# NethermindEth/zinc

Hardware: AMD Instinct MI355X
Metric: Zip commit+open MCoeffs/s at 2^24 witness (higher is better)
Workload: dtype i64

## Files before the change

zinc_amd/csrc/kernels_commit.cuh:

```cuda
#pragma once
#include <hip/hip_runtime.h>
#include <stdint.h>

#include "blake3.cuh"

namespace zipk {

typedef __int128 i128;
typedef unsigned __int128 u128;

#ifdef ZIPK_DEBUG_STAMPS
constexpr uint32_t kStampRec = 64;
__device__ __forceinline__ unsigned long long stamp_hw_id() {
    const uint32_t xcc = __builtin_amdgcn_s_getreg((3 << 11) | 20), hw = __builtin_amdgcn_s_getreg((31 << 11) | 4);
    return (unsigned long long)xcc | ((unsigned long long)hw << 8);
}
#endif

struct CommitArgs {
    const int64_t *evals;
    const uint32_t *perm1;
    const uint32_t *perm2;
    uint64_t *rows;
    uint32_t compact_rows;
// ... 162 lines not shown
    template <int E0>
    __device__ __forceinline__ void store_row_of(uint32_t d0, uint32_t d1, uint32_t d2) {
        if (MASKED && !(smask & (1u << E0))) return;
        const uint32_t j = base + E0 * T + tid;
        const uint32_t s = (uint32_t)((int32_t)d2 >> 31);
        if (MODE == kStorePacked) {
            const uint32_t pos = pbase<E0>() + lanes_below(__builtin_amdgcn_ballot_w64(true));
            *reinterpret_cast<uint4 *>(pk_v + (size_t)pos * 64) = make_uint4(d0, d1, d2, s);
        } else if (compact) {
            *reinterpret_cast<uint4 *>(out_row + (size_t)j * 2) = make_uint4(d0, d1, d2, s);
        } else {
            uint4 *o = reinterpret_cast<uint4 *>(out_row + (size_t)j * 4);
            o[0] = make_uint4(d0, d1, d2, s);
            o[1] = make_uint4(s, s, s, s);
        }
    }
    template <int E0>
    __device__ __forceinline__ void store_row() {
        uint32_t d0, d1, d2;
        entry<E0>(d0, d1, d2);
        store_row_of<E0>(d0, d1, d2);
    }
    template <int E0>
    __device__ __forceinline__ void leaf(uint32_t (&h)[8]) {
        uint32_t d0, d1, d2;
        entry<E0>(d0, d1, d2);
        store_row_of<E0>(d0, d1, d2);
        blake3_leaf_sext96(d0, d1, d2, h);
        if (!MASKED || (smask & (0x100u << E0))) {
            if (MODE == kStorePacked) {
                const uint32_t pos = pbase<8 + E0>() + lanes_below(__builtin_amdgcn_ballot_w64(true));
                store_hash(reinterpret_cast<uint32_t *>(pk_n + pk_off0) + (size_t)pos * 32, h);
            } else {
                store_hash(tree + (size_t)(base + E0 * T + tid) * 8, h);
            }
        }
    }
    template <int LVL, int E0>
    __device__ __forceinline__ void store(const uint32_t (&h)[8]) {
        if (MASKED && LVL <= 2 && !(smask & ((LVL == 1 ? 0x10000u : 0x1000000u) << (E0 >> LVL)))) return;
        const uint32_t e = E0 + (tid & ((1u << LVL) - 1u));
        const uint32_t n = (base + e * T + tid) >> LVL;
        if (MODE == kStorePacked && LVL == 1) {
            const uint64_t act = __builtin_amdgcn_ballot_w64(true);
            const bool odd = tid & 1u;
            const uint32_t pos = (odd ? pbase<16 + (E0 >> 1) * 2 + 1>() : pbase<16 + (E0 >> 1) * 2>()) +
                                 lanes_below(act & (odd ? 0xAAAAAAAAAAAAAAAAull : 0x5555555555555555ull));
            store_hash(reinterpret_cast<uint32_t *>(pk_n + pk_off1) + (size_t)pos * 32, h);
        } else if (MODE == kStorePacked && LVL == 2) {
            const uint64_t act = __builtin_amdgcn_ballot_w64(true);
            const uint32_t q = tid & 3u;
            constexpr int K0 = 24 + ((E0 >> 2) & 1) * 4;
            const uint32_t b01 = (q & 1u) ? pbase<K0 + 1>() : pbase<K0>(), b23 = (q & 1u) ? pbase<K0 + 3>() : pbase<K0 + 2>();
            const uint32_t pos = ((q & 2u) ? b23 : b01) + lanes_below(act & (0x1111111111111111ull << q));
            store_hash(reinterpret_cast<uint32_t *>(pk_n + pk_off2) + (size_t)pos * 32, h);
        } else {
            store_hash(tree + ((size_t)level_off(cw, LVL) + n) * NW, h);
        }
    }
};

template <int E>
__device__ __forceinline__ uint32_t store_mask(const uint32_t *need, uint32_t cw, uint32_t base, uint32_t T, uint32_t tid) {
    if (!need) return 0xFFFFFFFFu;
    const uint32_t *nv = need, *n0 = nv + (cw + 31) / 32, *n1 = n0 + (cw + 31) / 32, *n2 = n1 + (cw / 2 + 31) / 32;
    uint32_t m = 0;
#pragma unroll
    for (int e = 0; e < E; e++) {
        const uint32_t j = base + e * T + tid;
        m |= ((nv[j >> 5] >> (j & 31)) & 1u) << e;
        m |= ((n0[j >> 5] >> (j & 31)) & 1u) << (8 + e);
    }
#pragma unroll
    for (int g = 0; g < E / 2; g++) {
        const uint32_t i = (base + (2 * g + (tid & 1u)) * T + tid) >> 1;
        m |= ((n1[i >> 5] >> (i & 31)) & 1u) << (16 + g);
    }
#pragma unroll
    for (int g = 0; g < E / 4; g++) {
        const uint32_t i = (base + (4 * g + (tid & 3u)) * T + tid) >> 2;
        m |= ((n2[i >> 5] >> (i & 31)) & 1u) << (24 + g);
    }
    return m;
}

template <int E, int E0, class Src>
__device__ __forceinline__ void store_rows_only(Src &src) {
    if constexpr (E0 < E) {
        src.template store_row<E0>();
        store_rows_only<E, E0 + 1>(src);
    }
}

template <int LVL, int E0, class Src>
__device__ __forceinline__ void bfly_hash(Src &src, uint32_t (&h)[8]) {
    if constexpr (LVL == 0) {
        src.template leaf<E0>(h);
    } else {
        uint32_t A[8], B[8], m[16];
        bfly_hash<LVL - 1, E0>(src, A);
        bfly_hash<LVL - 1, E0 + (1 << (LVL - 1))>(src, B);
        const bool up = (src.tid >> (LVL - 1)) & 1;
#pragma unroll
        for (int i = 0; i < 8; i++) {
            const uint32_t snd = up ? A[i] : B[i];
            const uint32_t rcv = __shfl_xor(snd, 1 << (LVL - 1), 64);
            m[i] = up ? rcv : A[i];
            m[8 + i] = up ? B[i] : rcv;
        }
        blake3_block64(m, h);
        src.template store<LVL, E0>(h);
    }
}

template <bool ILV>
__device__ __forceinline__ void upper_stage(const CommitArgs &a, uint32_t first, uint32_t nrows_c, uint32_t lvl, uint32_t nl,
                                            uint32_t lane, uint32_t nlanes) {
    constexpr uint32_t NW = kNodeWords<ILV>;
    const uint32_t cw = a.cw, depth = 31u - __builtin_clz(cw);
    const uint32_t u_shift = depth - (lvl - 1u) - nl;
    const uint32_t total = nrows_c << u_shift;
    const uint32_t slot0 = round_slot(blockIdx.x, gridDim.x, a.classes);
    for (uint32_t idx = lane; idx < total; idx += nlanes) {
        const uint32_t ri = idx >> u_shift, i = idx & ((1u << u_shift) - 1u);
        const uint32_t r = slot0 + (first + ri) * gridDim.x;
        uint32_t *tree = tree_of<ILV>(a.layers, cw, r);
        const uint32_t *ch = tree + ((size_t)level_off(cw, lvl - 1u) + ((size_t)i << nl)) * NW;
        uint32_t c0[8], c1[8], h0[8];
        load_hash(ch, c0);
        load_hash(ch + NW, c1);
        if (nl == 1u) {
            blake3_node(c0, c1, h0);
            store_hash(tree + ((size_t)level_off(cw, lvl) + i) * NW, h0);
            if (lvl == depth) store_hash(a.roots + (size_t)r * 8, h0);
        } else {
            uint32_t c2[8], c3[8], h1[8], h2[8];
            blake3_node(c0, c1, h0);
            uint32_t *o = tree + ((size_t)level_off(cw, lvl) + 2u * i) * NW;
            store_hash(o, h0);
            asm volatile("" ::: "memory");
            load_hash(ch + 2 * NW, c2);
            load_hash(ch + 3 * NW, c3);
            blake3_node(c2, c3, h1);
            store_hash(o + NW, h1);
            blake3_node(h0, h1, h2);
            store_hash(tree + ((size_t)level_off(cw, lvl + 1u) + i) * NW, h2);
            if (lvl + 1u == depth) store_hash(a.roots + (size_t)r * 8, h2);
        }
    }
}

struct ChunkCursor {
    uint32_t first = 0, index = 0;
    __device__ __forceinline__ bool ends_with(const CommitArgs &a, uint32_t round, bool last) const {
        if (last) return true;
        if (a.chunk_ends) return (a.chunk_ends >> round) & 1u;
        return (round + 1) % a.rounds_per_chunk == 0;
    }
    __device__ __forceinline__ void advance(uint32_t round) {
        first = round + 1;
        index++;
    }
};

constexpr uint32_t kFinisherFlagWords = 16;

// ... 106 lines not shown
            __syncthreads();
            uint4 *in = bufA, *out = bufB;
            for (uint32_t lvl = p_lvl; lvl <= depth; lvl++) {
                const uint32_t w = cw >> lvl, sh = 31u - __builtin_clz(w), m = p_nrows * w;
                for (uint32_t idx = tid; idx < m; idx += T) {
                    const uint32_t ri = idx >> sh, i = idx & (w - 1u);
                    const uint32_t r = slot0 + (p_first + ri) * gridDim.x;
                    const uint4 a0 = in[4u * idx], a1 = in[4u * idx + 1u], b0 = in[4u * idx + 2u], b1 = in[4u * idx + 3u];
                    const uint32_t c0[8] = {a0.x, a0.y, a0.z, a0.w, a1.x, a1.y, a1.z, a1.w};
                    const uint32_t c1[8] = {b0.x, b0.y, b0.z, b0.w, b1.x, b1.y, b1.z, b1.w};
                    uint32_t h[8];
                    blake3_node(c0, c1, h);
                    store_hash(tree_of<ILV>(a.layers, cw, r) + ((size_t)level_off(cw, lvl) + i) * NW, h);
                    if (lvl == depth) store_hash(a.roots + (size_t)r * 8, h);
                    out[2u * idx] = make_uint4(h[0], h[1], h[2], h[3]);
                    out[2u * idx + 1u] = make_uint4(h[4], h[5], h[6], h[7]);
                }
                __syncthreads();
                uint4 *t = in;
                in = out;
                out = t;
            }
            if (wave == 0u) publish(a, p_index, lane);
            return;
        }
        after_hash(a, wave, lane, T);
    }

    __device__ __forceinline__ void chunk_end(const CommitArgs &a, uint32_t first_level, const ChunkCursor &cc, uint32_t round,
                                              bool last, uint32_t tid, uint32_t T) {
        const uint32_t wave = __builtin_amdgcn_readfirstlane(tid >> 6), lane = tid & 63u;
        if (!HASH) {
            if (a.chunk_done) {
                __syncthreads();
                if (wave == 0) publish(a, cc.index, lane);
            }
            return;
        }
        const uint32_t cw = a.cw, depth = 31u - __builtin_clz(cw);
        const uint32_t first = cc.first, nrows_c = round - first + 1;
        uint32_t lvl = first_level;
        const bool now = last || lvl > depth;
        if (now) {
            __syncthreads();
            if (lvl <= depth) {
                const uint32_t nl = depth - lvl >= 1u ? 2u : 1u;
                upper_stage<ILV>(a, first, nrows_c, lvl, nl, tid, T);
                lvl += nl;
            }
        }
        if (depth == 0 && tid == 0) {
            for (uint32_t ri = 0; ri < nrows_c; ri++) {
                const uint32_t r = round_slot(blockIdx.x, gridDim.x, a.classes) + (first + ri) * gridDim.x;
                uint32_t h[8];
                load_hash(a.layers + (size_t)r * (2u * cw) * 8, h);
                store_hash(a.roots + (size_t)r * 8, h);
            }
        }
        if (!last) p_base = lvl;
        pending = true;
        p_first = first;
        p_nrows = nrows_c;
        p_lvl = lvl;
        p_index = cc.index;
    }
};

__device__ __forceinline__ void stamp_clock(const CommitArgs &a, int slot) {
    if (a.clock && blockIdx.x == 0 && threadIdx.x == 0) {
        a.clock[2 * slot] = __builtin_amdgcn_s_memtime();
        a.clock[2 * slot + 1] = __builtin_amdgcn_s_memrealtime();
    }
}

__device__ __forceinline__ uint32_t opaque_zero(uint32_t dep) {
    uint32_t z;
    asm volatile("s_mov_b32 %0, 0" : "=s"(z) : "s"(dep));
    return z;
}

template <int E, bool HASH, int MODE = kStoreAll>
__global__ void __launch_bounds__(1024, 4) raa_commit_kernel(CommitArgs a) {
    constexpr bool MASKED = MODE != kStoreAll;
    extern __shared__ __align__(16) unsigned char smem[];
    constexpr int LOGE = (E == 1) ? 0 : (E == 2) ? 1 : (E == 4) ? 2 : 3;
    static_assert((1 << LOGE) == E && E <= 8, "E must be 1, 2, 4 or 8");

    const uint32_t tid0 = threadIdx.x, T = blockDim.x;
    constexpr uint32_t PAD = 32 / E;
    const uint32_t PS = T + PAD;
    const uint32_t cw = a.cw, row_len = a.row_len;
    const bool active = tid0 < a.nact;
    stamp_clock(a, 0);

    i128 *wave_tot = reinterpret_cast<i128 *>(smem);
    uint64_t *t2lo = reinterpret_cast<uint64_t *>(smem + 512);
    uint32_t *t2hi = reinterpret_cast<uint32_t *>(t2lo + E * PS);
    int64_t *rowbuf = reinterpret_cast<int64_t *>(t2hi + E * PS);
    uint32_t pidx[E];
    auto load_pidx = [&](uint32_t t) {
#pragma unroll
        for (int e = 0; e < E; e++) {
            uint32_t v1 = 0, v2 = 0;
            if (active) {
                v1 = a.perm1[t * E + e] & (row_len - 1);
                const uint32_t p2 = a.perm2[t * E + e];
                v2 = (p2 & (E - 1)) * PS + (p2 >> LOGE);
            }
            pidx[e] = v1 | (v2 << 16);
        }
    };
    load_pidx(tid0);
    const uint32_t smask = (MASKED && active) ? store_mask<E>(a.need, cw, 0u, a.nact, tid0) : 0xFFFFFFFFu;
    uint32_t ptab[16] = {};
    if (MODE == kStorePacked) {
        const uint32_t *wt = a.pk_tab + (size_t)__builtin_amdgcn_readfirstlane(tid0 >> 6) * 16;
#pragma unroll
        for (int k = 0; k < 16; k++) ptab[k] = __builtin_amdgcn_readfirstlane(wt[k]);
    }
    constexpr int NPF = (E >= 2) ? E / 2 : 1;
    const bool prefetch = row_len == NPF * T;
    int64_t nxt[NPF];

#ifdef ZIPK_DEBUG_STAMPS
    unsigned long long ph_a = 0, ph_b = 0, ph_c = 0, ph_t;
    if (tid0 == 0 && a.stamps) {
        a.stamps[(size_t)kStampRec * blockIdx.x] = wall_clock64();
        a.stamps[(size_t)kStampRec * blockIdx.x + 2] = stamp_hw_id();
    }
#define ZIPK_PH(acc) do { const unsigned long long now_ = wall_clock64(); acc += now_ - ph_t; ph_t = now_; } while (0)
#else
#define ZIPK_PH(acc) do { } while (0)
#endif
    uint32_t round = 0;
    ChunkCursor cc;
    if (a.classes > 1u) {
        const uint32_t c = commit_class(blockIdx.x, gridDim.x, a.classes);
        cc.index = c;
        const uint32_t prio = (a.classes - 1u - c) * 3u / (a.classes - 1u);
        if (prio == 3u) __builtin_amdgcn_s_setprio(3);
        else if (prio == 2u) __builtin_amdgcn_s_setprio(2);
        else if (prio == 1u) __builtin_amdgcn_s_setprio(1);
    }
    ChunkFinisher<HASH, MODE == kStorePacked> fin;
    fin.init(reinterpret_cast<uint32_t *>(rowbuf + row_len), tid0);
    const uint32_t wave0 = __builtin_amdgcn_readfirstlane(tid0 >> 6);
    for (uint32_t row = round_slot(blockIdx.x, gridDim.x, a.classes); row < a.num_rows; row += gridDim.x, round++) {
#ifdef ZIPK_DEBUG_STAMPS
        ph_t = wall_clock64();
#endif
        const uint32_t z = opaque_zero(row);
        const uint32_t tid = tid0 + z;
        const int64_t *in = a.evals + (size_t)row * row_len;
        uint64_t *out_row = a.rows + (size_t)row * cw * (a.compact_rows ? 2 : 4);

        const bool has_next = row + gridDim.x < a.num_rows;
        if (!(prefetch && round)) {
            if (round) lds_barrier();
            for (uint32_t i = tid; i < row_len; i += T) rowbuf[i] = in[i];
            lds_barrier();
        }
        if (prefetch && has_next) {
            const int64_t *nin = a.evals + (size_t)(row + gridDim.x) * row_len;
#pragma unroll
            for (int k = 0; k < NPF; k++) nxt[k] = nin[k * T + tid];
        }

        i128 v[E];
        if (active) {
#pragma unroll
            for (int e = 0; e < E; e++) v[e] = (i128)rowbuf[(pidx[e] ^ z) & 0xFFFFu];
#pragma unroll
            for (int e = 1; e < E; e++) v[e] += v[e - 1];
        } else {
#pragma unroll
            for (int e = 0; e < E; e++) v[e] = 0;
        }
        {
            const i128 pre = block_exclusive_scan_i96(v[E - 1], wave_tot, 0);
            if (active) {
#pragma unroll
                for (int e = 0; e < E; e++) {
                    v[e] += pre;
                    const uint32_t slot = e * PS + tid;
                    t2lo[slot] = (uint64_t)v[e];
                    t2hi[slot] = (uint32_t)((u128)v[e] >> 64);
                }
            }
        }
        lds_barrier();
        if (active) {
#pragma unroll
            for (int e = 0; e < E; e++) {
                const uint32_t slot = (pidx[e] ^ z) >> 16;
                const uint64_t lo = t2lo[slot];
                const int64_t hi = (int64_t)(int32_t)t2hi[slot];
                v[e] = (i128)(((u128)(uint64_t)hi << 64) | lo);
            }
#pragma unroll
            for (int e = 1; e < E; e++) v[e] += v[e - 1];
        }
        {
            const i128 pre = block_exclusive_scan_i96(v[E - 1], wave_tot, 1);
#pragma unroll
            for (int e = 0; e < E; e++) v[e] += pre;
        }

        if (active) {
#pragma unroll
            for (int e = 0; e < E; e++) {
                const uint32_t slot = e * PS + tid;
                t2lo[slot] = (uint64_t)v[e];
                t2hi[slot] = (uint32_t)((u128)v[e] >> 64);
            }
        }
        if (prefetch && has_next) {
#pragma unroll
            for (int k = 0; k < NPF; k++) rowbuf[k * T + tid] = nxt[k];
        }
        fin.top_of_row();
        lds_barrier();
        ZIPK_PH(ph_a);
        if (active) {
            StridedLeaves<E, MODE, true> src;
            src.out_row = out_row;
            src.compact = a.compact_rows;
            src.tree = HASH ? tree_of<MODE == kStorePacked>(a.layers, cw, row) : nullptr;
            src.cw = cw;
            src.T = a.nact;
            src.tid = tid;
            src.smask = smask;
            if (MODE == kStorePacked) {
                src.set_packed(a, row);
#pragma unroll
                for (int k = 0; k < 16; k++) src.ptab[k] = ptab[k];
            }
            {
                const uint32_t slot0 = (tid & (E - 1)) * PS + (tid >> LOGE);
                src.lz_lo = t2lo + slot0;
                src.lz_hi = t2hi + slot0;
                src.lz_stride = a.nact >> LOGE;
            }
            if (HASH) {
                uint32_t top[8];
                bfly_hash<LOGE, 0>(src, top);
            } else {
                store_rows_only<E, 0>(src);
            }
        }
        ZIPK_PH(ph_b);
        fin.after_hash(a, wave0, tid0 & 63u, T);
        const bool last = row + gridDim.x >= a.num_rows;
        if (cc.ends_with(a, round, last)) {
            fin.chunk_end(a, LOGE + 1, cc, round, last, tid, T);
            cc.advance(round);
        }
        ZIPK_PH(ph_c);
#ifdef ZIPK_DEBUG_STAMPS
        if (tid0 == 0 && a.stamps && round < kStampRec - 8) a.stamps[(size_t)kStampRec * blockIdx.x + 8 + round] = ph_t;
#endif
    }
    fin.after_loop(a, wave0, tid0 & 63u, T, smem + 512, (uint32_t)(E * PS * 12u));
    stamp_clock(a, 1);
#ifdef ZIPK_DEBUG_STAMPS
    if (tid0 == 0 && a.stamps) {
        unsigned long long *o = a.stamps + (size_t)kStampRec * blockIdx.x;
        o[1] = wall_clock64();
        o[3] = ph_a; o[4] = ph_b; o[5] = ph_c; o[6] = round;
    }
#endif
}

constexpr size_t c16_lds_bytes(uint32_t T) {
    return 512 + (size_t)16 * (T + 2) * 8 + (size_t)16 * (T + 2) + (size_t)T * 4 + 64;
}

template <int B, int P = 0>
__device__ __forceinline__ void transpose8_stage(uint32_t (&x)[8], bool up) {
    if constexpr (P < 4) {
        constexpr int r = ((P >> B) << (B + 1)) | (P & ((1 << B) - 1)), r2 = r | (1 << B);
        const uint32_t lo = x[r], hi = x[r2];
        const uint32_t rcv = __shfl_xor(up ? lo : hi, 1 << B, 64);
        x[r] = up ? rcv : lo;
        x[r2] = up ? hi : rcv;
        transpose8_stage<B, P + 1>(x, up);
    }
}
__device__ __forceinline__ void transpose8(uint32_t (&x)[8], uint32_t lane) {
    transpose8_stage<0>(x, lane & 1u);
    transpose8_stage<1>(x, (lane >> 1) & 1u);
    transpose8_stage<2>(x, (lane >> 2) & 1u);
}

template <uint32_t T, bool HASH, int MODE = kStoreAll>
__global__ void __launch_bounds__(T, 4) raa_commit16_kernel(CommitArgs a) {
    constexpr bool MASKED = MODE != kStoreAll;
    static_assert(MODE == kStoreAll || MODE == kStoreHinted || MODE == kStorePacked, "store mode");
    extern __shared__ __align__(16) unsigned char smem[];
    constexpr int E = 16;
    constexpr uint32_t PS = T + 2;
    const uint32_t tid0 = threadIdx.x;
    const uint32_t cw = a.cw, row_len = a.row_len;
    stamp_clock(a, 0);

    i128 *wave_tot = reinterpret_cast<i128 *>(smem);
    uint64_t *t2lo = reinterpret_cast<uint64_t *>(smem + 512);
    int8_t *t2dh = reinterpret_cast<int8_t *>(t2lo + (size_t)E * PS);
    int32_t *ghi = reinterpret_cast<int32_t *>(t2dh + (size_t)E * PS);
    uint64_t *park_lo = reinterpret_cast<uint64_t *>(smem + 512);
    uint32_t *park_hi = reinterpret_cast<uint32_t *>(park_lo + (size_t)8 * PS);

    const uint32_t smask0 = MASKED ? store_mask<8>(a.need, cw, 0u, 16u, (tid0 & ~7u) * 16u + (tid0 & 7u)) : 0xFFFFFFFFu;
    const uint32_t smask1 = MASKED ? store_mask<8>(a.need, cw, 0u, 16u, (tid0 & ~7u) * 16u + 8u + (tid0 & 7u)) : 0xFFFFFFFFu;
    uint32_t ptab0[16] = {}, ptab1[16] = {};
    if (MODE == kStorePacked) {
        const uint32_t *wt = a.pk_tab + (size_t)__builtin_amdgcn_readfirstlane(tid0 >> 6) * 32;
#pragma unroll
        for (int k = 0; k < 16; k++) {
            ptab0[k] = __builtin_amdgcn_readfirstlane(wt[k]);
// ... 369 lines not shown
```

zinc_amd/csrc/zip_hip.hip:

```cpp
#include <hip/hip_runtime.h>
#include <dlfcn.h>
#include <algorithm>
#include <atomic>
#include <chrono>
#include <thread>

#include <climits>
#include <cstdarg>
#include <cstdio>
#include <cstdlib>
#include <cstring>
#include <functional>
#include <map>
#include <memory>
#include <mutex>
#include <new>
#include <string>
#include <vector>

#include "../../include/zip_hip.h"
#include "kernels_commit.cuh"
#include "kernels_open.cuh"
#include "kernels_batch.cuh"
#include "kernels_verify.cuh"
#include "kernels_batch_verify.cuh"
#include "kernels_sumcheck.cuh"
#include "kernels_sumcheck_tail.cuh"
#include "kernels_sumcheck_wide.cuh"
#include "kernels_spartan.cuh"
#include "rccl_dyn.h"

using namespace zipk;

namespace {

typedef unsigned __int128 u128;

bool is_pow2(uint64_t x) { return x && !(x & (x - 1)); }
uint32_t ilog2(uint64_t x) { return 63u - (uint32_t)__builtin_clzll(x); }

long env_long(const char *name, long def, long lo, long hi) {
    const char *e = getenv(name);
    if (!e) return def;
    char *end = nullptr;
    const long v = strtol(e, &end, 10);
    return end == e || v < lo || v > hi ? def : v;
}

struct KernelStat {
    uint32_t launches = 0;
    float total_ms = 0.f;
};
struct PendingEvent {
    const char *name;
    hipEvent_t start, stop;
};

}

struct PackedLayout {
    uint32_t stride = 0, off[3] = {};
};
struct HintPlan {
    uint32_t cw = 0, e = 0, threads = 0;
    bool want_packed = false;
    std::vector<uint32_t> cols;
    std::vector<uint32_t> bm;
    bool packed = false;
    PackedLayout L;
    std::vector<uint32_t> wave_tab;
    std::vector<uint16_t> pos[4];
    std::vector<uint16_t> own_ranks;
    unsigned char *dev = nullptr;
    std::function<void(unsigned char *)> release;
    HintPlan() = default;
    HintPlan(const HintPlan &) = delete;
    HintPlan &operator=(const HintPlan &) = delete;
    ~HintPlan() { if (dev && release) release(dev); }
    bool ranks(const uint32_t *cs, uint32_t n, uint16_t *out) const {
        for (uint32_t i = 0; i < n; i++) {
            const uint32_t col = cs[i];
            if (col >= cw) return false;
            const uint16_t r[4] = {pos[0][col], pos[1][col ^ 1u], pos[2][(col >> 1) ^ 1u], pos[3][(col >> 2) ^ 1u]};
            for (int k = 0; k < 4; k++) {
                if (r[k] == 0xFFFF) return false;
                out[4 * i + k] = r[k];
            }
        }
        return true;
    }
};

static inline int speculation_default_flag() {
    const long v = env_long("ZIP_HIP_SPECULATE", -1, 0, 1);
    return v < 0 ? 1 : v == 0 ? 0 : 2;
}

struct zip_ctx {
    zip_params p{};
    uint32_t depth = 0;
    uint32_t rows_local = 0;
    int device = 0;
    hipStream_t stream = nullptr, s_commit = nullptr, s_upper = nullptr;
    uint32_t n_chunks = 1;
    uint32_t knob_rpb = 0;
    int knob_stream = -1;
    std::string knob_chunk_rounds;
    bool no_compact = false;
    uint32_t num_cus = 256;
    uint32_t *timeout_flag_h = nullptr, *timeout_flag_d = nullptr;
    unsigned long long *clock_h = nullptr, *clock_d = nullptr;
    std::vector<hipEvent_t> dep_event_pool;
    uint32_t *perm1_d = nullptr, *perm2_d = nullptr;
    unsigned char *pinned_base = nullptr, *stage_h = nullptr, *stage_big = nullptr;
    size_t stage_cap = 0, stage_big_cap = 0;
    unsigned char *bounce[2] = {nullptr, nullptr};
    size_t bounce_cap = 0;
    std::vector<unsigned char *> hint_free;
    std::shared_ptr<bool> alive = std::make_shared<bool>(true);
    bool profile_commit_only = false;
    std::shared_ptr<HintPlan> hint_plan;
    int speculate = speculation_default_flag();
    bool seen_columns = false;
    uint32_t *ring_d = nullptr;
    uint32_t ring_next = 0, ring_epoch = 0;
    uint4 *slab_d = nullptr;
    size_t slab_bytes = 0;
    unsigned char *job_stage[2] = {nullptr, nullptr};
    size_t job_stage_cap[2] = {0, 0};
    bool job_busy[2] = {false, false};
    uint64_t recover_epoch = 0;
    zip_field field_cache_in{};
    alignas(8) unsigned char field_cache_out[256] = {};
    bool field_cache_valid = false;
    std::string last_error;
    bool recycle = false;
    size_t h2d_bounce_threshold = (size_t)8 << 20;
    std::multimap<size_t, void *> free_blocks;
    std::map<void *, size_t> live_blocks;
    std::mutex mu;
    std::recursive_mutex api_mu;
    bool profiling = false;
    std::vector<PendingEvent> pending;
    std::vector<hipEvent_t> event_pool;
    std::map<std::string, KernelStat> stats;
    std::vector<std::string> stat_names;
};

struct BatchStore {
    void *rows = nullptr, *layers = nullptr, *roots = nullptr, *evals = nullptr;
    std::function<void(BatchStore &)> release;
    BatchStore() = default;
    BatchStore(const BatchStore &) = delete;
// ... 567 lines not shown
    return ZIP_OK;
}

template <int FL>
FieldDev<FL> to_dev(const HostField &h) {
    FieldDev<FL> d;
    for (int i = 0; i < FL; i++) {
        d.modulus[i] = h.modulus[i];
        d.r2[i] = h.r2[i];
    }
    d.inv = h.inv;
    return d;
}

int32_t ensure_dynamic_lds(zip_ctx *ctx, const void *kern, size_t bytes) {
    static std::mutex mu;
    static std::map<std::pair<const void *, int>, size_t> granted;
    std::lock_guard<std::mutex> g(mu);
    size_t &have = granted[std::make_pair(kern, ctx->device)];
    if (bytes > have) {
        HIP_TRY(ctx, hipFuncSetAttribute(kern, hipFuncAttributeMaxDynamicSharedMemorySize, (int)bytes));
        have = bytes;
    }
    return ZIP_OK;
}

template <int E, bool HASH, int MODE = kStoreAll>
int32_t launch_commit(zip_ctx *ctx, const CommitArgs &a, uint32_t threads, uint32_t grid, hipStream_t st) {
    size_t lds = 512 + (size_t)E * (threads + 32 / E) * 12 + (size_t)a.row_len * 8 + 4 * kFinisherFlagWords;
    auto kern = raa_commit_kernel<E, HASH, MODE>;
    if (int32_t rc = ensure_dynamic_lds(ctx, reinterpret_cast<const void *>(kern), lds)) return rc;
    LaunchTimer t(ctx, HASH ? "raa_commit_kernel" : "raa_encode_kernel", st);
    hipLaunchKernelGGL(kern, dim3(grid), dim3(threads), lds, st, a);
    HIP_TRY(ctx, hipGetLastError());
    return ZIP_OK;
}

template <bool HASH, int MODE = kStoreAll>
int32_t launch_commit16(zip_ctx *ctx, const CommitArgs &a, uint32_t grid, hipStream_t st) {
    constexpr uint32_t T = 1024;
    auto kern = raa_commit16_kernel<T, HASH, MODE>;
    if (int32_t rc = ensure_dynamic_lds(ctx, reinterpret_cast<const void *>(kern), c16_lds_bytes(T))) return rc;
    LaunchTimer t(ctx, HASH ? "raa_commit_kernel" : "raa_encode_kernel", st);
    hipLaunchKernelGGL(kern, dim3(grid), dim3(T), c16_lds_bytes(T), st, a);
    HIP_TRY(ctx, hipGetLastError());
    return ZIP_OK;
}

template <bool HASH>
int32_t launch_commit_slab(zip_ctx *ctx, const CommitArgs &a, uint32_t grid, hipStream_t st) {
    auto kern = a.cw == 65536 ? raa_commit_slab_kernel<64, HASH> : raa_commit_slab_kernel<32, HASH>;
    if (int32_t rc = ensure_dynamic_lds(ctx, reinterpret_cast<const void *>(kern), cslab_lds_bytes())) return rc;
    LaunchTimer t(ctx, HASH ? "raa_commit_kernel" : "raa_encode_kernel", st);
    hipLaunchKernelGGL(kern, dim3(grid), dim3(kSlabThreads), cslab_lds_bytes(), st, a);
    HIP_TRY(ctx, hipGetLastError());
    return ZIP_OK;
}

struct CommitGeom {
    uint32_t e, threads;
    size_t lds;
};
CommitGeom commit_geom(uint32_t cw, uint32_t row_len) {
    CommitGeom g{};
    if (cw >= 32768) { g.e = cw / kSlabThreads; g.threads = kSlabThreads; g.lds = cslab_lds_bytes(); return g; }
    if (cw == 16384) { g.e = 16; g.threads = 1024; g.lds = c16_lds_bytes(1024); return g; }
    if (cw >= 512) { g.e = 8; g.threads = cw / 8; }
    else if (cw == 256) { g.e = 4; g.threads = 64; }
    else if (cw == 128) { g.e = 2; g.threads = 64; }
    else { g.e = 1; g.threads = 64; }
    g.lds = 512 + (size_t)g.e * (g.threads + 32 / g.e) * 12 + (size_t)row_len * 8 + 4 * kFinisherFlagWords;
    return g;
}
uint32_t commit_wgs_per_cu(const CommitGeom &g) {
    if (g.e > 16) return 1;
    uint32_t by_threads = 2048 / g.threads, by_lds = (uint32_t)((160u * 1024u) / g.lds);
    uint32_t k = by_threads < by_lds ? by_threads : by_lds;
    if (k > 8) k = 8;
    return k ? k : 1;
}

bool commit_supports_hint(uint32_t cw) { return cw >= 512 && cw <= 16384; }
constexpr uint32_t kRingSlots = 64, kRingChunks = 16, kRingStride = 16;
constexpr size_t kHintTables = 8192, kHintBytes = kHintTables + 8 * (8192 / 32) + 4 * 4096 + 64, kPackedRanksAt = kHintTables + 2048;
static bool packed_enabled() {
    return env_long("ZIP_HIP_PACKED", 1, 0, 1) != 0;
}
static void plan_packed(HintPlan &P) {
    const uint32_t cw = P.cw, wv = (cw + 31) / 32, w1 = (cw / 2 + 31) / 32;
    const uint32_t *sec[4] = {P.bm.data(), P.bm.data() + wv, P.bm.data() + 2 * wv, P.bm.data() + 2 * wv + w1};
    const uint32_t bits[4] = {cw, cw, cw / 2, cw / 4};
    const uint32_t waves = P.threads / 64, phases = P.e == 16 ? 2 : 1, sT = P.e == 16 ? 16 : P.threads;
    for (int k = 0; k < 4; k++) P.pos[k].assign(bits[k], 0xFFFF);
    P.wave_tab.assign((size_t)waves * phases * 16, 0);
    uint32_t cnt[4] = {0, 0, 0, 0};
    auto member = [&](int k, uint32_t i) { return (sec[k][i >> 5] >> (i & 31u)) & 1u; };
    for (uint32_t w = 0; w < waves; w++)
        for (uint32_t q = 0; q < phases; q++) {
            uint16_t base[32];
            auto stid = [&](uint32_t l) {
                const uint32_t tid = 64 * w + l;
                return P.e == 16 ? (tid & ~7u) * 16u + q * 8u + (tid & 7u) : tid;
            };
            auto site = [&](int k, int slot, uint32_t step, uint32_t shift, uint32_t cls, uint32_t ncls) {
                base[slot] = (uint16_t)cnt[k];
                for (uint32_t l = cls; l < 64; l += ncls) {
                    const uint32_t i = (step * sT + stid(l)) >> shift;
                    if (member(k, i)) P.pos[k][i] = (uint16_t)cnt[k]++;
                }
            };
            for (uint32_t e = 0; e < 8; e++) site(0, (int)e, e, 0, 0, 1);
            for (uint32_t e = 0; e < 8; e++) site(1, (int)(8 + e), e, 0, 0, 1);
            for (uint32_t g = 0; g < 4; g++)
                for (uint32_t par = 0; par < 2; par++) site(2, (int)(16 + 2 * g + par), 2 * g + par, 1, par, 2);
            for (uint32_t g = 0; g < 2; g++)
                for (uint32_t c4 = 0; c4 < 4; c4++) site(3, (int)(24 + 4 * g + c4), 4 * g + c4, 2, c4, 4);
            uint32_t *tab = P.wave_tab.data() + ((size_t)w * phases + q) * 16;
            for (uint32_t k = 0; k < 16; k++) tab[k] = (uint32_t)base[2 * k] | ((uint32_t)base[2 * k + 1] << 16);
        }
    uint32_t at = (cnt[0] * 16u + 127u) & ~127u;
    P.L.off[0] = at;
    at = (at + cnt[1] * 32u + 127u) & ~127u;
    P.L.off[1] = at;
    at = (at + cnt[2] * 32u + 127u) & ~127u;
    P.L.off[2] = at;
    at = (at + cnt[3] * 32u + 127u) & ~127u;
    P.L.stride = at;
}
static std::shared_ptr<HintPlan> get_hint_plan(zip_ctx *ctx, const uint32_t *cols, uint32_t n_cols, bool want_packed) {
    const uint32_t cw = ctx->p.codeword_len;
    const CommitGeom g = commit_geom(cw, ctx->p.row_len);
    if (ctx->hint_plan) {
        const HintPlan &h = *ctx->hint_plan;
        if (h.cw == cw && h.e == g.e && h.threads == g.threads && h.want_packed == want_packed && h.cols.size() == n_cols &&
            (n_cols == 0 || !memcmp(h.cols.data(), cols, (size_t)n_cols * 4)))
            return ctx->hint_plan;
    }
    auto P = std::make_shared<HintPlan>();
    P->cw = cw;
    P->e = g.e;
    P->threads = g.threads;
    P->want_packed = want_packed;
    P->cols.assign(cols, cols + n_cols);
    const uint32_t wv = (cw + 31) / 32, w1 = (cw / 2 + 31) / 32, w2 = (cw / 4 + 31) / 32;
    P->bm.assign(2 * (size_t)wv + w1 + w2, 0);
    uint32_t *nv = P->bm.data(), *n0 = nv + wv, *n1 = n0 + wv, *n2 = n1 + w1;
    for (uint32_t i = 0; i < n_cols; i++) {
        const uint32_t col = cols[i];
        nv[col >> 5] |= 1u << (col & 31);
        const uint32_t s0 = col ^ 1u, s1 = (col >> 1) ^ 1u, s2 = (col >> 2) ^ 1u;
        n0[s0 >> 5] |= 1u << (s0 & 31);
        n1[s1 >> 5] |= 1u << (s1 & 31);
        n2[s2 >> 5] |= 1u << (s2 & 31);
    }
    if (want_packed && n_cols && (g.e == 8 || g.e == 16) && cw >= 512 && g.threads % 64 == 0 && cw == g.e * g.threads &&
        ctx->depth >= 3) {
        plan_packed(*P);
        P->own_ranks.resize((size_t)n_cols * 4);
        P->packed = P->L.stride > 0 && P->wave_tab.size() * 4 <= kPackedRanksAt - kHintTables &&
                    kPackedRanksAt + P->own_ranks.size() * 2 <= kHintBytes && P->ranks(cols, n_cols, P->own_ranks.data());
    }
    std::vector<unsigned char> img(kHintBytes, 0);
    memcpy(img.data(), P->bm.data(), P->bm.size() * 4);
    size_t used = P->bm.size() * 4;
    if (P->packed) {
        memcpy(img.data() + kHintTables, P->wave_tab.data(), P->wave_tab.size() * 4);
        memcpy(img.data() + kPackedRanksAt, P->own_ranks.data(), P->own_ranks.size() * 2);
        used = kPackedRanksAt + P->own_ranks.size() * 2;
    }
    void *blk = nullptr;
    if (used <= kHintBytes && pool_alloc(ctx, kHintBytes, &blk) == ZIP_OK) {
        if (hipMemcpy(blk, img.data(), used, hipMemcpyHostToDevice) == hipSuccess) {
            P->dev = static_cast<unsigned char *>(blk);
            std::shared_ptr<bool> alive = ctx->alive;
            P->release = [ctx, alive](unsigned char *p) { if (*alive) pool_release(ctx, p); };
        } else {
            pool_release(ctx, blk);
            (void)hipGetLastError();
        }
    }
    ctx->hint_plan = P;
    return P;
}

template <bool HASH>
int32_t dispatch_commit(zip_ctx *ctx, CommitArgs a, uint32_t grid, hipStream_t st) {
    const CommitGeom g = commit_geom(a.cw, a.row_len);
    a.nact = a.cw / g.e < g.threads ? a.cw / g.e : g.threads;
    if (HASH && a.need) {
        if (g.e == 8 && a.pk) return launch_commit<8, HASH, HASH ? kStorePacked : kStoreAll>(ctx, a, g.threads, grid, st);
        if (g.e == 16 && a.pk) return launch_commit16<HASH, HASH ? kStorePacked : kStoreAll>(ctx, a, grid, st);
        a.pk = nullptr;
        if (g.e == 16) return launch_commit16<HASH, HASH ? kStoreHinted : kStoreAll>(ctx, a, grid, st);
        if (g.e == 8) return launch_commit<8, HASH, HASH ? kStoreHinted : kStoreAll>(ctx, a, g.threads, grid, st);
        a.need = nullptr;
    }
    a.pk = nullptr;
    switch (g.e) {
        case 64:
        case 32: return launch_commit_slab<HASH>(ctx, a, grid, st);
        case 16: return launch_commit16<HASH>(ctx, a, grid, st);
        case 8: return launch_commit<8, HASH>(ctx, a, g.threads, grid, st);
        case 4: return launch_commit<4, HASH>(ctx, a, g.threads, grid, st);
        case 2: return launch_commit<2, HASH>(ctx, a, g.threads, grid, st);
        default: return launch_commit<1, HASH>(ctx, a, g.threads, grid, st);
    }
}

template <int NL>
int32_t launch_upper(zip_ctx *ctx, hipStream_t st, uint32_t *layers, uint32_t *roots, uint32_t trees, uint32_t cw,
                     uint32_t level_in, uint32_t depth) {
    const uint64_t total = (uint64_t)trees * ((cw >> level_in) >> NL);
    const uint32_t threads = 256;
    const uint32_t blocks = (uint32_t)((total + threads - 1) / threads);
    LaunchTimer t(ctx, "merkle_upper_kernel", st);
    hipLaunchKernelGGL(merkle_upper_kernel<NL>, dim3(blocks), dim3(threads), 0, st, layers, roots, trees, cw,
                       level_in, depth);
    HIP_TRY(ctx, hipGetLastError());
    return ZIP_OK;
}

int32_t merkle_upper_levels(zip_ctx *ctx, hipStream_t st, uint32_t *layers, uint32_t *roots, uint32_t trees,
                            uint32_t cw, uint32_t level, uint32_t depth) {
    if (depth == 0) {
        LaunchTimer t(ctx, "copy_roots_depth0_kernel", st);
        hipLaunchKernelGGL(copy_roots_depth0_kernel, dim3((trees + 255) / 256), dim3(256), 0, st, layers, roots,
                           trees, cw);
        HIP_TRY(ctx, hipGetLastError());
        return ZIP_OK;
    }
    while (level < depth) {
        const uint32_t rem = depth - level;
        int32_t rc;
        if (rem >= 4) {
            rc = launch_upper<4>(ctx, st, layers, roots, trees, cw, level, depth);
            level += 4;
        } else if (rem == 3) {
            rc = launch_upper<3>(ctx, st, layers, roots, trees, cw, level, depth);
            level += 3;
        } else if (rem == 2) {
            rc = launch_upper<2>(ctx, st, layers, roots, trees, cw, level, depth);
            level += 2;
        } else {
            rc = launch_upper<1>(ctx, st, layers, roots, trees, cw, level, depth);
            level += 1;
        }
        if (rc) return rc;
    }
    return ZIP_OK;
// ... 1233 lines not shown
                    sched.push_back(last);
                }
            }
        }
        uint64_t chunk_ends = 0;
        if (sched.empty()) {
            for (uint32_t k = 0; k < nch; k++) sched.push_back(std::min(rpc, rounds - k * rpc));
        } else {
            nch = (uint32_t)sched.size();
            uint32_t r = 0;
            for (uint32_t k = 0; k < nch; k++) {
                r += sched[k];
                chunk_ends |= 1ull << (r - 1);
            }
        }
        c->bounds.resize(nch + 1);
        {
            uint64_t r = 0;
            for (uint32_t k = 0; k <= nch; k++) {
                const uint64_t b = r * G;
                c->bounds[k] = b < R ? (uint32_t)b : R;
                if (k < nch) r += sched[k];
            }
        }
        uint32_t classes = 1;
        {
            const long knob_classes = env_long("ZIP_HIP_CLASSES", 0, 1, 64);
            const uint32_t per_cu = commit_wgs_per_cu(geom);
            if (with_merkle && hint_cols && commit_supports_hint(cw) && rounds == 1 && R == G && per_cu >= 2 && G % 8 == 0 &&
                !ctx->n_chunks && knob_classes != 1) {
                classes = knob_classes > 1 ? (uint32_t)knob_classes : std::min(2u, per_cu);
                while (classes > 1 && ((G / 8) % classes || classes > per_cu)) classes--;
            }
            if (classes > 1) {
                nch = classes;
                chunk_ends = 0;
                c->bounds.resize(nch + 1);
                for (uint32_t k = 0; k <= nch; k++) c->bounds[k] = k * (G / classes);
            }
        }
        CommitArgs a{};
        a.classes = classes;
        a.evals = evals_d;
        a.perm1 = ctx->perm1_d;
        a.perm2 = ctx->perm2_d;
        a.rows = c->rows;
        a.compact_rows = c->compact_rows ? 1u : 0u;
        a.layers = c->layers;
        a.row_len = C;
        a.cw = cw;
        a.num_rows = R;
        a.rounds_per_chunk = rpc;
        a.chunk_ends = chunk_ends;
        a.roots = c->roots;
        a.clock = ctx->profiling ? ctx->clock_d : nullptr;
#ifdef ZIPK_DEBUG_STAMPS
        a.stamps = debug_stamps_buffer();
#endif
        hipError_t e = hipSuccess;
        if (with_merkle && hint_cols && commit_supports_hint(cw)) {
            const uint32_t wv = (cw + 31) / 32, w1 = (cw / 2 + 31) / 32, w2 = (cw / 4 + 31) / 32;
            const size_t words = 2 * (size_t)wv + w1 + w2;
            if (words * 4 > kHintBytes) { rc = fail(ctx, ZIP_ERR_UNSUPPORTED, "hint bitmaps exceed their staging block"); break; }
            const bool want_packed = c->compact_rows && n_hint && packed_enabled();
            c->plan = get_hint_plan(ctx, hint_cols, n_hint, want_packed);
            const bool resident = c->plan->dev != nullptr;
            if (!resident) {
                if (!ctx->hint_free.empty()) {
                    c->hint_h = ctx->hint_free.back();
                    ctx->hint_free.pop_back();
                } else if (hipHostMalloc((void **)&c->hint_h, kHintBytes, hipHostMallocDefault) != hipSuccess) {
                    c->hint_h = nullptr;
                    rc = fail(ctx, ZIP_ERR_ALLOC, "hipHostMalloc(%zu) failed", kHintBytes);
                    break;
                }
            }
            uint32_t *bm = resident ? nullptr : reinterpret_cast<uint32_t *>(c->hint_h);
            if (bm) memcpy(bm, c->plan->bm.data(), words * 4);
            const uint32_t *nv = c->plan->bm.data();
            c->hint_cols.assign(nv, nv + wv);
            size_t upload = words * 4;
            if (c->plan->packed) {
                if (!resident) {
                    memcpy(c->hint_h + kHintTables, c->plan->wave_tab.data(), c->plan->wave_tab.size() * 4);
                    memcpy(c->hint_h + kPackedRanksAt, c->plan->own_ranks.data(), c->plan->own_ranks.size() * 2);
                }
                upload = kPackedRanksAt + c->plan->own_ranks.size() * 2;
                c->packed = true;
                c->pk_stride = c->plan->L.stride;
                for (int k = 0; k < 3; k++) c->pk_off[k] = c->plan->L.off[k];
            }
            const unsigned char *tables_d;
            if (resident) {
                tables_d = c->plan->dev;
            } else {
                if ((rc = pool_alloc(ctx, kHintBytes, (void **)&c->need_d))) break;
                e = hipMemcpyAsync(c->need_d, bm, upload, hipMemcpyHostToDevice, ctx->s_commit);
                if (e != hipSuccess) { rc = fail(ctx, ZIP_ERR_HIP, "hint upload failed: %s", hipGetErrorString(e)); break; }
                tables_d = reinterpret_cast<const unsigned char *>(c->need_d);
            }
            a.need = reinterpret_cast<const uint32_t *>(tables_d);
            c->hinted = true;
            if (c->packed) {
                a.pk = reinterpret_cast<uint8_t *>(c->rows);
                a.pk_stride = c->pk_stride;
                a.pk_off0 = c->pk_off[0];
                a.pk_off1 = c->pk_off[1];
                a.pk_off2 = c->pk_off[2];
                a.pk_tab = reinterpret_cast<const uint32_t *>(tables_d + kHintTables);
                c->rank_d = reinterpret_cast<const uint16_t *>(tables_d + kPackedRanksAt);
            }
        }
        if (with_merkle && (nch > 1 || (hint_cols && R >= ctx->num_cus))) {
            if (nch <= kRingChunks && !ctx->ring_d) {
                if (hipMalloc((void **)&ctx->ring_d, (size_t)kRingSlots * kRingStride * 4) != hipSuccess ||
                    hipMemset(ctx->ring_d, 0, (size_t)kRingSlots * kRingStride * 4) != hipSuccess) {
                    if (ctx->ring_d) (void)hipFree(ctx->ring_d);
                    ctx->ring_d = nullptr;
                    (void)hipGetLastError();
                }
            }
            if (nch <= kRingChunks && ctx->ring_d) {
                if (ctx->ring_next == kRingSlots) {
                    if (e == hipSuccess) e = stream_wait(ctx->stream);
                    if (e == hipSuccess) e = stream_wait(ctx->s_commit);
                    if (e == hipSuccess) e = hipMemsetAsync(ctx->ring_d, 0, (size_t)kRingSlots * kRingStride * 4, ctx->s_commit);
                    if (e == hipSuccess) e = stream_wait(ctx->s_commit);
                    ctx->ring_next = 0;
                    ctx->ring_epoch++;
                }
                c->chunk_done = ctx->ring_d + (size_t)ctx->ring_next++ * kRingStride;
                c->ring_slot = true;
                c->ring_epoch = ctx->ring_epoch;
            } else {
                if ((rc = pool_alloc(ctx, (size_t)nch * 4, (void **)&c->chunk_done))) break;
                e = hipMemsetAsync(c->chunk_done, 0, (size_t)nch * 4, ctx->s_commit);
                c->zeroed = take_dep_event(ctx);
                if (e == hipSuccess) e = hipEventRecord(c->zeroed, ctx->s_commit);
            }
            a.chunk_done = c->chunk_done;
            c->expected.resize(nch);
            for (uint32_t k = 0; k < nch; k++) c->expected[k] = (R - c->bounds[k]) < G ? (R - c->bounds[k]) : G;
            if (classes > 1)
                for (uint32_t k = 0; k < nch; k++) c->expected[k] = G / classes;
        }
        if (e != hipSuccess) { rc = fail(ctx, ZIP_ERR_HIP, "commit setup failed: %s", hipGetErrorString(e)); break; }
        if (geom.e > 16) {
            const size_t need = (size_t)G * cw * 16;
            if (ctx->slab_bytes < need) {
                if (ctx->slab_d && (e = stream_wait(ctx->s_commit)) != hipSuccess) {
                    rc = fail(ctx, ZIP_ERR_HIP, "commit setup failed: %s", hipGetErrorString(e));
                    break;
                }
                if (ctx->slab_d) (void)hipFree(ctx->slab_d);
                ctx->slab_d = nullptr;
                ctx->slab_bytes = 0;
                if (hipMalloc((void **)&ctx->slab_d, need) != hipSuccess) {
                    ctx->slab_d = nullptr;
                    (void)hipGetLastError();
                    rc = fail(ctx, ZIP_ERR_ALLOC, "hipMalloc(%zu) of the commit slabs failed", need);
                    break;
                }
                ctx->slab_bytes = need;
            }
            a.slab = ctx->slab_d;
        }
        rc = with_merkle ? dispatch_commit<true>(ctx, a, G, ctx->s_commit) : dispatch_commit<false>(ctx, a, G, ctx->s_commit);
// ... 2196 lines not shown
```

Before: 11030.

## Give packed E=8 commits contiguous per-thread leaf ownership with own-subtree hashing

For the packed store mode with eight entries per thread, each thread now hashes its own contiguous eight leaves as a depth-3 subtree. It places packed leaf and node outputs using per-thread rank prefixes (two words per thread) in place of per-wave strided tables. The host planner gains a matching per-thread rank layout and a larger rank-table region, while the strided-16 path is kept for E=16. The work before the last barrier is moved under the scan's barrier and the extra LDS barrier before hashing is dropped, saving a block-wide sync per row. This relies on the scan barrier also covering the transposed LDS writes, and it changes the hint image layout.

```diff
diff --git a/zinc_amd/csrc/kernels_commit.cuh b/zinc_amd/csrc/kernels_commit.cuh
--- a/zinc_amd/csrc/kernels_commit.cuh
+++ b/zinc_amd/csrc/kernels_commit.cuh
@@ -268,6 +268,78 @@
         m |= ((n2[i >> 5] >> (i & 31)) & 1u) << (24 + g);
     }
     return m;
+}
+
+struct OwnLeaves8 {
+    const uint64_t *lz_lo;
+    const uint32_t *lz_hi;
+    uint32_t lz_stride;
+    uint32_t *node3;
+    uint8_t *pk_v, *pk_n;
+    uint32_t pk_off0, pk_off1, pk_off2;
+    uint32_t rk01, rk23;
+    uint32_t smask;
+    __device__ __forceinline__ void set_packed(const CommitArgs &a, uint32_t row) {
+        uint8_t *g = a.pk + (size_t)(row >> 2) * 4 * a.pk_stride;
+        pk_v = g + (row & 3u) * 16u;
+        pk_n = g + (row & 3u) * 32u;
+        pk_off0 = 4u * a.pk_off0;
+        pk_off1 = 4u * a.pk_off1;
+        pk_off2 = 4u * a.pk_off2;
+    }
+    template <int B, int S>
+    __device__ __forceinline__ uint32_t place(uint32_t base) const {
+        return base + (uint32_t)__builtin_popcount(smask & (((1u << B) - 1u) & ~((1u << S) - 1u)));
+    }
+    template <int E0>
+    __device__ __forceinline__ void leaf(uint32_t (&h)[8]) {
+        const uint64_t lo = lz_lo[E0 * lz_stride];
+        const uint32_t d0 = (uint32_t)lo, d1 = (uint32_t)(lo >> 32), d2 = lz_hi[E0 * lz_stride];
+        if (smask & (1u << E0)) {
+            const uint32_t pos = place<E0, 0>(rk01 & 0xFFFFu);
+            *reinterpret_cast<uint4 *>(pk_v + (size_t)pos * 64) = make_uint4(d0, d1, d2, (uint32_t)((int32_t)d2 >> 31));
+        }
+        blake3_leaf_sext96(d0, d1, d2, h);
+        if (smask & (0x100u << E0)) {
+            const uint32_t pos = place<8 + E0, 8>(rk01 >> 16);
+            store_hash(reinterpret_cast<uint32_t *>(pk_n + pk_off0) + (size_t)pos * 32, h);
+        }
+    }
+    template <int LVL, int I>
+    __device__ __forceinline__ void node(const uint32_t (&h)[8]) {
+        if constexpr (LVL == 1) {
+            if (smask & (0x10000u << I)) {
+                const uint32_t pos = place<16 + I, 16>(rk23 & 0xFFFFu);
+                store_hash(reinterpret_cast<uint32_t *>(pk_n + pk_off1) + (size_t)pos * 32, h);
+            }
+        } else if constexpr (LVL == 2) {
+            if (smask & (0x1000000u << I)) {
+                const uint32_t pos = place<24 + I, 24>(rk23 >> 16);
+                store_hash(reinterpret_cast<uint32_t *>(pk_n + pk_off2) + (size_t)pos * 32, h);
+            }
+        } else {
+            store_hash(node3, h);
+        }
+    }
+    __device__ __forceinline__ void store(int lvl, uint32_t idx, const uint32_t (&h)[8]) {
+        if (lvl == 1) {
+            if (idx == 0) node<1, 0>(h);
+            else if (idx == 1) node<1, 1>(h);
+            else if (idx == 2) node<1, 2>(h);
+            else node<1, 3>(h);
+        } else if (lvl == 2) {
+            if (idx == 0) node<2, 0>(h);
+            else node<2, 1>(h);
+        } else {
+            node<3, 0>(h);
+        }
+    }
+};
+
+__device__ __forceinline__ uint32_t store_mask_own8(const uint32_t *need, uint32_t cw, uint32_t tid) {
+    const uint32_t *nv = need, *n0 = nv + (cw + 31) / 32, *n1 = n0 + (cw + 31) / 32, *n2 = n1 + (cw / 2 + 31) / 32;
+    return ((nv[tid >> 2] >> ((tid & 3u) * 8u)) & 0xFFu) | (((n0[tid >> 2] >> ((tid & 3u) * 8u)) & 0xFFu) << 8) |
+           (((n1[tid >> 3] >> ((tid & 7u) * 4u)) & 0xFu) << 16) | (((n2[tid >> 4] >> ((tid & 15u) * 2u)) & 3u) << 24);
 }
 
 template <int E, int E0, class Src>
@@ -540,9 +612,11 @@
 template <int E, bool HASH, int MODE = kStoreAll>
 __global__ void __launch_bounds__(1024, 4) raa_commit_kernel(CommitArgs a) {
     constexpr bool MASKED = MODE != kStoreAll;
+    constexpr bool OWN = MODE == kStorePacked;
     extern __shared__ __align__(16) unsigned char smem[];
     constexpr int LOGE = (E == 1) ? 0 : (E == 2) ? 1 : (E == 4) ? 2 : 3;
     static_assert((1 << LOGE) == E && E <= 8, "E must be 1, 2, 4 or 8");
+    static_assert(!OWN || (E == 8 && HASH), "packed commits of this kernel: 8 entries per thread, hashed");
 
     const uint32_t tid0 = threadIdx.x, T = blockDim.x;
     constexpr uint32_t PAD = 32 / E;
@@ -569,12 +643,14 @@
         }
     };
     load_pidx(tid0);
-    const uint32_t smask = (MASKED && active) ? store_mask<E>(a.need, cw, 0u, a.nact, tid0) : 0xFFFFFFFFu;
-    uint32_t ptab[16] = {};
-    if (MODE == kStorePacked) {
-        const uint32_t *wt = a.pk_tab + (size_t)__builtin_amdgcn_readfirstlane(tid0 >> 6) * 16;
-#pragma unroll
-        for (int k = 0; k < 16; k++) ptab[k] = __builtin_amdgcn_readfirstlane(wt[k]);
+    const uint32_t smask = !(MASKED && active) ? 0xFFFFFFFFu
+                           : OWN               ? store_mask_own8(a.need, cw, tid0)
+                                               : store_mask<E>(a.need, cw, 0u, a.nact, tid0);
+    uint32_t rk01 = 0, rk23 = 0;
+    if (OWN && active) {
+        const uint2 rk = reinterpret_cast<const uint2 *>(a.pk_tab)[tid0];
+        rk01 = rk.x;
+        rk23 = rk.y;
     }
     constexpr int NPF = (E >= 2) ? E / 2 : 1;
     const bool prefetch = row_len == NPF * T;
@@ -658,6 +734,14 @@
 #pragma unroll
             for (int e = 1; e < E; e++) v[e] += v[e - 1];
         }
+        auto under_last_barrier = [&]() {
+            if (prefetch && has_next) {
+#pragma unroll
+                for (int k = 0; k < NPF; k++) rowbuf[k * T + tid] = nxt[k];
+            }
+            fin.top_of_row();
+        };
+        if (OWN) under_last_barrier();
         {
             const i128 pre = block_exclusive_scan_i96(v[E - 1], wave_tot, 1);
 #pragma unroll
@@ -672,27 +756,36 @@
                 t2hi[slot] = (uint32_t)((u128)v[e] >> 64);
             }
         }
-        if (prefetch && has_next) {
-#pragma unroll
-            for (int k = 0; k < NPF; k++) rowbuf[k * T + tid] = nxt[k];
-        }
-        fin.top_of_row();
-        lds_barrier();
+        if (OWN) {
+            asm volatile("" ::: "memory");
+        } else {
+            under_last_barrier();
+            lds_barrier();
+        }
         ZIPK_PH(ph_a);
-        if (active) {
+        if constexpr (OWN) {
+            if (active) {
+                OwnLeaves8 src;
+                src.lz_lo = t2lo + tid;
+                src.lz_hi = t2hi + tid;
+                src.lz_stride = PS;
+                src.node3 = tree_of<true>(a.layers, cw, row) + ((size_t)level_off(cw, 3) + tid) * kNodeWords<true>;
+                src.set_packed(a, row);
+                src.rk01 = rk01 ^ z;
+                src.rk23 = rk23 ^ z;
+                src.smask = smask ^ z;
+                uint32_t top[8];
+                subtree_hash<3, 0>(src, top);
+            }
+        } else if (active) {
             StridedLeaves<E, MODE, true> src;
             src.out_row = out_row;
             src.compact = a.compact_rows;
-            src.tree = HASH ? tree_of<MODE == kStorePacked>(a.layers, cw, row) : nullptr;
+            src.tree = HASH ? tree_of<false>(a.layers, cw, row) : nullptr;
             src.cw = cw;
             src.T = a.nact;
             src.tid = tid;
             src.smask = smask;
-            if (MODE == kStorePacked) {
-                src.set_packed(a, row);
-#pragma unroll
-                for (int k = 0; k < 16; k++) src.ptab[k] = ptab[k];
-            }
             {
                 const uint32_t slot0 = (tid & (E - 1)) * PS + (tid >> LOGE);
                 src.lz_lo = t2lo + slot0;
diff --git a/zinc_amd/csrc/zip_hip.hip b/zinc_amd/csrc/zip_hip.hip
--- a/zinc_amd/csrc/zip_hip.hip
+++ b/zinc_amd/csrc/zip_hip.hip
@@ -68,7 +68,7 @@
     std::vector<uint32_t> bm;
     bool packed = false;
     PackedLayout L;
-    std::vector<uint32_t> wave_tab;
+    std::vector<uint32_t> rank_tab;
     std::vector<uint16_t> pos[4];
     std::vector<uint16_t> own_ranks;
     unsigned char *dev = nullptr;
@@ -802,31 +802,65 @@
 
 bool commit_supports_hint(uint32_t cw) { return cw >= 512 && cw <= 16384; }
 constexpr uint32_t kRingSlots = 64, kRingChunks = 16, kRingStride = 16;
-constexpr size_t kHintTables = 8192, kHintBytes = kHintTables + 8 * (8192 / 32) + 4 * 4096 + 64, kPackedRanksAt = kHintTables + 2048;
+constexpr size_t kHintTables = 8192, kPackedRanksAt = kHintTables + 8192, kHintBytes = kPackedRanksAt + 8 * (8192 / 32) + 4 * 4096 + 64;
 static bool packed_enabled() {
     return env_long("ZIP_HIP_PACKED", 1, 0, 1) != 0;
 }
-static void plan_packed(HintPlan &P) {
-    const uint32_t cw = P.cw, wv = (cw + 31) / 32, w1 = (cw / 2 + 31) / 32;
-    const uint32_t *sec[4] = {P.bm.data(), P.bm.data() + wv, P.bm.data() + 2 * wv, P.bm.data() + 2 * wv + w1};
-    const uint32_t bits[4] = {cw, cw, cw / 2, cw / 4};
-    const uint32_t waves = P.threads / 64, phases = P.e == 16 ? 2 : 1, sT = P.e == 16 ? 16 : P.threads;
-    for (int k = 0; k < 4; k++) P.pos[k].assign(bits[k], 0xFFFF);
-    P.wave_tab.assign((size_t)waves * phases * 16, 0);
+static void packed_layout(HintPlan &P, const uint32_t (&cnt)[4]) {
+    uint32_t at = (cnt[0] * 16u + 127u) & ~127u;
+    P.L.off[0] = at;
+    at = (at + cnt[1] * 32u + 127u) & ~127u;
+    P.L.off[1] = at;
+    at = (at + cnt[2] * 32u + 127u) & ~127u;
+    P.L.off[2] = at;
+    at = (at + cnt[3] * 32u + 127u) & ~127u;
+    P.L.stride = at;
+}
+struct HintSections {
+    const uint32_t *sec[4];
+    uint32_t bits[4];
+    explicit HintSections(const HintPlan &P) {
+        const uint32_t cw = P.cw, wv = (cw + 31) / 32, w1 = (cw / 2 + 31) / 32;
+        const uint32_t *b = P.bm.data();
+        sec[0] = b, sec[1] = b + wv, sec[2] = b + 2 * wv, sec[3] = b + 2 * wv + w1;
+        bits[0] = cw, bits[1] = cw, bits[2] = cw / 2, bits[3] = cw / 4;
+    }
+    uint32_t member(int k, uint32_t i) const { return (sec[k][i >> 5] >> (i & 31u)) & 1u; }
+};
+static void plan_packed_own8(HintPlan &P) {
+    const HintSections S(P);
+    for (int k = 0; k < 4; k++) P.pos[k].assign(S.bits[k], 0xFFFF);
     uint32_t cnt[4] = {0, 0, 0, 0};
-    auto member = [&](int k, uint32_t i) { return (sec[k][i >> 5] >> (i & 31u)) & 1u; };
+    P.rank_tab.assign((size_t)P.threads * 2, 0);
+    for (uint32_t t = 0; t < P.threads; t++) {
+        P.rank_tab[2 * t] = cnt[0] | (cnt[1] << 16);
+        P.rank_tab[2 * t + 1] = cnt[2] | (cnt[3] << 16);
+        for (int k = 0; k < 4; k++) {
+            const uint32_t per = S.bits[k] / P.threads;
+            for (uint32_t i = t * per; i < (t + 1) * per; i++)
+                if (S.member(k, i)) P.pos[k][i] = (uint16_t)cnt[k]++;
+        }
+    }
+    packed_layout(P, cnt);
+}
+static void plan_packed_strided16(HintPlan &P) {
+    const HintSections S(P);
+    const uint32_t waves = P.threads / 64, phases = 2, sT = 16;
+    for (int k = 0; k < 4; k++) P.pos[k].assign(S.bits[k], 0xFFFF);
+    P.rank_tab.assign((size_t)waves * phases * 16, 0);
+    uint32_t cnt[4] = {0, 0, 0, 0};
     for (uint32_t w = 0; w < waves; w++)
         for (uint32_t q = 0; q < phases; q++) {
             uint16_t base[32];
             auto stid = [&](uint32_t l) {
                 const uint32_t tid = 64 * w + l;
-                return P.e == 16 ? (tid & ~7u) * 16u + q * 8u + (tid & 7u) : tid;
+                return (tid & ~7u) * 16u + q * 8u + (tid & 7u);
             };
             auto site = [&](int k, int slot, uint32_t step, uint32_t shift, uint32_t cls, uint32_t ncls) {
                 base[slot] = (uint16_t)cnt[k];
                 for (uint32_t l = cls; l < 64; l += ncls) {
                     const uint32_t i = (step * sT + stid(l)) >> shift;
-                    if (member(k, i)) P.pos[k][i] = (uint16_t)cnt[k]++;
+                    if (S.member(k, i)) P.pos[k][i] = (uint16_t)cnt[k]++;
                 }
             };
             for (uint32_t e = 0; e < 8; e++) site(0, (int)e, e, 0, 0, 1);
@@ -835,17 +869,14 @@
                 for (uint32_t par = 0; par < 2; par++) site(2, (int)(16 + 2 * g + par), 2 * g + par, 1, par, 2);
             for (uint32_t g = 0; g < 2; g++)
                 for (uint32_t c4 = 0; c4 < 4; c4++) site(3, (int)(24 + 4 * g + c4), 4 * g + c4, 2, c4, 4);
-            uint32_t *tab = P.wave_tab.data() + ((size_t)w * phases + q) * 16;
+            uint32_t *tab = P.rank_tab.data() + ((size_t)w * phases + q) * 16;
             for (uint32_t k = 0; k < 16; k++) tab[k] = (uint32_t)base[2 * k] | ((uint32_t)base[2 * k + 1] << 16);
         }
-    uint32_t at = (cnt[0] * 16u + 127u) & ~127u;
-    P.L.off[0] = at;
-    at = (at + cnt[1] * 32u + 127u) & ~127u;
-    P.L.off[1] = at;
-    at = (at + cnt[2] * 32u + 127u) & ~127u;
-    P.L.off[2] = at;
-    at = (at + cnt[3] * 32u + 127u) & ~127u;
-    P.L.stride = at;
+    packed_layout(P, cnt);
+}
+static void plan_packed(HintPlan &P) {
+    if (P.e == 8) plan_packed_own8(P);
+    else plan_packed_strided16(P);
 }
 static std::shared_ptr<HintPlan> get_hint_plan(zip_ctx *ctx, const uint32_t *cols, uint32_t n_cols, bool want_packed) {
     const uint32_t cw = ctx->p.codeword_len;
@@ -877,14 +908,14 @@
         ctx->depth >= 3) {
         plan_packed(*P);
         P->own_ranks.resize((size_t)n_cols * 4);
-        P->packed = P->L.stride > 0 && P->wave_tab.size() * 4 <= kPackedRanksAt - kHintTables &&
+        P->packed = P->L.stride > 0 && P->rank_tab.size() * 4 <= kPackedRanksAt - kHintTables &&
                     kPackedRanksAt + P->own_ranks.size() * 2 <= kHintBytes && P->ranks(cols, n_cols, P->own_ranks.data());
     }
     std::vector<unsigned char> img(kHintBytes, 0);
     memcpy(img.data(), P->bm.data(), P->bm.size() * 4);
     size_t used = P->bm.size() * 4;
     if (P->packed) {
-        memcpy(img.data() + kHintTables, P->wave_tab.data(), P->wave_tab.size() * 4);
+        memcpy(img.data() + kHintTables, P->rank_tab.data(), P->rank_tab.size() * 4);
         memcpy(img.data() + kPackedRanksAt, P->own_ranks.data(), P->own_ranks.size() * 2);
         used = kPackedRanksAt + P->own_ranks.size() * 2;
     }
@@ -2284,7 +2315,7 @@
             size_t upload = words * 4;
             if (c->plan->packed) {
                 if (!resident) {
-                    memcpy(c->hint_h + kHintTables, c->plan->wave_tab.data(), c->plan->wave_tab.size() * 4);
+                    memcpy(c->hint_h + kHintTables, c->plan->rank_tab.data(), c->plan->rank_tab.size() * 4);
                     memcpy(c->hint_h + kPackedRanksAt, c->plan->own_ranks.data(), c->plan->own_ranks.size() * 2);
                 }
                 upload = kPackedRanksAt + c->plan->own_ranks.size() * 2;
```

Measured after the change: 11280, median of 6. 2.3% higher.
